# mmSir/SpatioTemporalEntropyModel

Measured on AMD Instinct MI355X. Metric: frames/s, higher is better.
Workload: dtype f32; 1 GPU; configs[1]: SpatioTemporalPriorModel_Res(256,192) training step on mbt2018(192,192) latents, 16 septuplets x 7 frames x 256x256 per GPU, EMLoss, clip 1.0 + Adam 1e-4 / aux Adam 1e-3; per_gpu_batch=16, global_batch=16, parallelism=dp1, stream_priorities=latents=0,side=-1,compute=-1, stream_cu_masks=latents=block:160, plan_selectors=library defaults

## Files before the change

### spatiotemporalentropymodel_amd/csrc/conv_f16x3.hip

```cpp
#include <math.h>
#include <stdlib.h>

#include <type_traits>

#include "f16x3_tail.h"

namespace {

constexpr int XP = BN + 4;
constexpr int imax(int a, int b) { return a > b ? a : b; }
constexpr int lds_stages(int depth) { return depth == 3 ? 3 : 2; }
constexpr int lds_taps(int bm, int depth) { return imax(imax(lds_stages(depth) * NPL * (bm + BN) * 64, 6 * NPL * bm * 64 + NPL * BN * 64), bm * XP * 4); }
constexpr int lds_total(int bm, int depth) { return lds_taps(bm, depth) + 32 * 4; }

struct Fx3Phase {
    int ntaps, S;
    int dy0, dx0;
    int wofs;
    int cps, nsplit;
    int wsofs;
    int ooy, oox;
};

struct Fx3Args {
// ... 17 lines not shown
    float *ws;
    int *cnt;
    int nsplit, cps;
    int xpix;
    signed char dy[MAXTAP], dx[MAXTAP];
    int ptiles, btaps, OHf, OWf;
    Fx3Phase ph[4];
};

#define TAP_OFFSET(t) (tw_first + ((t) / tw_S) * tw_line + ((t) % tw_S) * tw_col)
#define TAP_WALK_NEXT()                                                                         \
    do {                                                                                        \
        const bool wrap_ = pf_t + 1 == tw_T, rowend_ = pf_ts + 1 == tw_S;                       \
        ++pf_q;                                                                                 \
        pf_to = wrap_ ? tw_first : pf_to + (rowend_ ? tw_line - (tw_S - 1) * tw_col : tw_col);  \
        pf_ts = (wrap_ || rowend_) ? 0 : pf_ts + 1;                                             \
        pf_t = wrap_ ? 0 : pf_t + 1;                                                            \
        pf_kc += wrap_ ? 1 : 0;                                                                 \
    } while (0)


__device__ inline int pi4(int x) { return (0x78 >> (2 * x)) & 3; }

template <int BM, int DEPTH, int MS>
__global__ __launch_bounds__(BM * 4) void conv_f16x3_kernel(const Fx3Args a)
{
    static_assert(DEPTH == 2 || DEPTH == 3, "two or three LDS stages");
    static_assert(MS == 32 || (MS == 16 && DEPTH == 3), "the 16-row MFMA shape exists for the three-stage loop");
    constexpr int NSET = 2;
    constexpr int NT = BM * 4;
    constexpr int A_PLANE = BM * 64, A_BUF = NPL * A_PLANE;
    constexpr int PL = NPL;
    constexpr int WPIECES = PL * BN * 4;
    constexpr int BP = (WPIECES + NT - 1) / NT;
    extern __shared__ __attribute__((aligned(16))) unsigned char smem[];
    constexpr int NST = lds_stages(DEPTH);
    unsigned char *As = smem;
    unsigned char *Bs = smem + NST * A_BUF;

    const int tid = threadIdx.x, lane = tid & 63, wave = tid >> 6;
    const int Mtot = a.B * a.OH * a.OW;
    int tile_m = blockIdx.x;
    {
        const int nb = gridDim.x, qq = nb >> 3, rr = nb & 7, xcd = tile_m & 7, idx = tile_m >> 3;
        if (nb >= 16) tile_m = (xcd < rr ? xcd * (qq + 1) : rr * (qq + 1) + (xcd - rr) * qq) + idx;
    }
    const int bm0 = tile_m * BM;
    const int nslab = a.C / KC, pixbytes = nslab * SLAB;

    const int srow = tid >> 2, scol = tid & 3;
    int pb;
    unsigned pmask = 0;
    {
        const int m = bm0 + srow;
        const bool ok = m < Mtot;
        const int mm = ok ? m : 0;
        const int ohw = a.OH * a.OW, b = mm / ohw, rem = mm - b * ohw, qy = rem / a.OW, qx = rem - qy * a.OW;
        const int by = qy * a.stride, bx = qx * a.stride;
        pb = ((b * a.H + by) * a.W + bx) * pixbytes + scol * 16;
        for (int t = 0; t < a.ntaps; ++t) {
            const int iy = by + a.dy[t], ix = bx + a.dx[t];
            if (ok && iy >= 0 && iy < a.H && ix >= 0 && ix < a.W) pmask |= 1u << t;
        }
    }
    const int a_st = srow * 64 + ((scol ^ ((srow >> 2) & 3)) << 4);
    constexpr int WFULL = WPIECES / NT;
    const int wv0 = tid * 16, wvl = WFULL * NT + tid < WPIECES ? (WFULL * NT + tid) * 16 : OOR;
    const int nchunks = a.ntaps * nslab;
    const int q_last = nchunks - 1;
    __syncthreads();

    const __amdgpu_buffer_rsrc_t rx = __builtin_amdgcn_make_buffer_rsrc(const_cast<void *>(a.xp), 0, a.xbytes, 0x00020000);
    const __amdgpu_buffer_rsrc_t rw = __builtin_amdgcn_make_buffer_rsrc(const_cast<void *>(a.wp), 0, a.wbytes, 0x00020000);

    f32x4 rsa[NSET][PL], rsb[NSET][BP];
    auto gload = [&](int t, int tA, int kc, int q, f32x4 (&ra)[PL], f32x4 (&rb)[BP]) {
        const int sA = kc * SLAB, sB = q * B_BUF;
        const int mk = __builtin_amdgcn_sbfe((int)pmask, (unsigned)t, 1u);
        const int off = ((pb + tA) & mk) | (OOR & ~mk);
#pragma unroll
        for (int pl = 0; pl < PL; ++pl) ra[pl] = __builtin_bit_cast(f32x4, __builtin_amdgcn_raw_buffer_load_b128(rx, off + pl * 64, sA, 0));
#pragma unroll
        for (int j = 0; j < WFULL; ++j)
            rb[j] = __builtin_bit_cast(f32x4, __builtin_amdgcn_raw_buffer_load_b128(rw, wv0 + j * (NT * 16), sB, 0));
        if (BP > WFULL) rb[BP - 1] = __builtin_bit_cast(f32x4, __builtin_amdgcn_raw_buffer_load_b128(rw, wvl, sB, 0));
    };
    auto sstore = [&](int buf, f32x4 (&ra)[PL], f32x4 (&rb)[BP]) {
#pragma unroll
        for (int pl = 0; pl < PL; ++pl) *reinterpret_cast<f32x4 *>(As + buf * A_BUF + pl * A_PLANE + a_st) = ra[pl];
#pragma unroll
        for (int j = 0; j < WFULL; ++j) *reinterpret_cast<f32x4 *>(Bs + buf * B_BUF + j * (NT * 16) + tid * 16) = rb[j];
        if (BP > WFULL && WFULL * NT + tid < WPIECES) *reinterpret_cast<f32x4 *>(Bs + buf * B_BUF + (WFULL * NT + tid) * 16) = rb[BP - 1];
    };

    const int wm0 = (wave >> 1) * 32, wn0 = (wave & 1) * 96;
    const int lr = lane & 31, lh = lane >> 5;
    const int sw = (lr >> 2) & 3;
    const int rdA = (wm0 + lr) * 64, rdB = (wn0 + lr) * 64;
    const int pk0 = ((0 + lh) ^ sw) << 4, pk1 = ((2 + lh) ^ sw) << 4;
    const int l16 = lane & 15, lq = lane >> 4;
    const int cm = 4 * pi4(l16 >> 2) + (l16 & 3), rq = 4 * pi4(lq);
    const int rdA16 = (wm0 + cm) * 64 + ((lq ^ pi4(l16 >> 2)) << 4), rdB16 = (wn0 + cm) * 64 + ((lq ^ pi4(l16 >> 2)) << 4);
    auto ROWL = [&](int r) { return MS == 32 ? wm0 + (r & 3) + 8 * (r >> 2) + 4 * lh : wm0 + ((r >> 2) & 1) * 16 + rq + (r & 3); };
    auto COLL = [&](int j, int r) { return MS == 32 ? wn0 + j * 32 + lr : wn0 + j * 32 + (r >> 3) * 16 + cm; };
    f32x16 acc[3];
#pragma unroll
    for (int j = 0; j < 3; ++j)
#pragma unroll
        for (int r = 0; r < 16; ++r) acc[j][r] = 0.f;

    int pf_q = 0, pf_t = 0, pf_kc = 0, pf_ts = 0, pf_to = 0;
    const int tw_T = a.ntaps, tw_S = a.S, tw_col = pixbytes, tw_line = a.W * pixbytes, tw_first = (a.dy[0] * a.W + a.dx[0]) * pixbytes;
    auto step = [&](int cur, f32x4 (&ra)[PL], f32x4 (&rb)[BP]) {
        const unsigned char *Ab = As + cur * A_BUF + rdA, *Bb = Bs + cur * B_BUF + rdB;
        const int t = __builtin_amdgcn_readfirstlane(pf_t), kc = __builtin_amdgcn_readfirstlane(pf_kc), q = __builtin_amdgcn_readfirstlane(pf_q);
        const int to = __builtin_amdgcn_readfirstlane(pf_to);
#pragma unroll
        for (int ks = 0; ks < 2; ++ks) {
            const int pk = ks ? pk1 : pk0;
            h16x8 af[PL], bf[PL][3];
#pragma unroll
            for (int pl = 0; pl < PL; ++pl) af[pl] = *reinterpret_cast<const h16x8 *>(Ab + pl * A_PLANE + pk);
#pragma unroll
            for (int pl = 0; pl < PL; ++pl)
#pragma unroll
                for (int j = 0; j < 3; ++j) bf[pl][j] = *reinterpret_cast<const h16x8 *>(Bb + pl * B_PLANE + j * 32 * 64 + pk);
#pragma unroll
            for (int j = 0; j < 3; ++j) {
                acc[j] = STEM_MFMA16(af[1], bf[0][j], acc[j]);
                acc[j] = STEM_MFMA16(af[0], bf[1][j], acc[j]);
                acc[j] = STEM_MFMA16(af[0], bf[0][j], acc[j]);
            }
            if (ks == 0)
                sstore(cur ^ 1, ra, rb);
            else
                gload(t, to, kc, q, ra, rb);
        }
        if (pf_q < q_last) TAP_WALK_NEXT();
    };
    h16x8 f0a[PL], f0b[PL][3], f1a[PL], f1b[PL][3];
    auto lfrag = [&](int stage, int pk, h16x8 (&af)[PL], h16x8 (&bf)[PL][3]) {
        const unsigned char *Ab = As + stage * A_BUF + rdA + pk, *Bb = Bs + stage * B_BUF + rdB + pk;
        af[1] = *reinterpret_cast<const h16x8 *>(Ab + A_PLANE);
        bf[0][0] = *reinterpret_cast<const h16x8 *>(Bb);
        af[0] = *reinterpret_cast<const h16x8 *>(Ab);
        bf[1][0] = *reinterpret_cast<const h16x8 *>(Bb + B_PLANE);
#pragma unroll
        for (int j = 1; j < 3; ++j) {
            bf[0][j] = *reinterpret_cast<const h16x8 *>(Bb + j * 32 * 64);
            bf[1][j] = *reinterpret_cast<const h16x8 *>(Bb + B_PLANE + j * 32 * 64);
        }
    };
    auto mfma9 = [&](h16x8 (&af)[PL], h16x8 (&bf)[PL][3]) {
#pragma unroll
        for (int j = 0; j < 3; ++j) {
            acc[j] = STEM_MFMA16(af[1], bf[0][j], acc[j]);
            acc[j] = STEM_MFMA16(af[0], bf[1][j], acc[j]);
            acc[j] = STEM_MFMA16(af[0], bf[0][j], acc[j]);
        }
    };
    auto step3 = [&](int rd, int nx, int wr, f32x4 (&ra)[PL], f32x4 (&rb)[BP]) {
        const int t = __builtin_amdgcn_readfirstlane(pf_t), kc = __builtin_amdgcn_readfirstlane(pf_kc), q = __builtin_amdgcn_readfirstlane(pf_q);
        const int to = __builtin_amdgcn_readfirstlane(pf_to);
        lfrag(rd, pk1, f1a, f1b);
        mfma9(f0a, f0b);
        sstore(wr, ra, rb);
        lfrag(nx, pk0, f0a, f0b);
        mfma9(f1a, f1b);
        gload(t, to, kc, q, ra, rb);
#pragma unroll
        for (int i = 0; i < 8; ++i) {
            __builtin_amdgcn_sched_group_barrier(0x008, 1, 0);
            __builtin_amdgcn_sched_group_barrier(0x100, 1, 0);
        }
        __builtin_amdgcn_sched_group_barrier(0x008, 1, 0);
        constexpr int NW = PL + BP;
        __builtin_amdgcn_sched_group_barrier(0x008, 1, 0);
        __builtin_amdgcn_sched_group_barrier(0x200, (NW + 3) / 4, 0);
        __builtin_amdgcn_sched_group_barrier(0x008, 1, 0);
        __builtin_amdgcn_sched_group_barrier(0x200, (NW + 2) / 4, 0);
        __builtin_amdgcn_sched_group_barrier(0x008, 1, 0);
        __builtin_amdgcn_sched_group_barrier(0x200, (NW + 1) / 4, 0);
        __builtin_amdgcn_sched_group_barrier(0x008, 1, 0);
        __builtin_amdgcn_sched_group_barrier(0x200, NW / 4, 0);
#pragma unroll
        for (int i = 0; i < 4; ++i) {
            __builtin_amdgcn_sched_group_barrier(0x008, 1, 0);
            __builtin_amdgcn_sched_group_barrier(0x100, 2, 0);
        }
        __builtin_amdgcn_sched_group_barrier(0x008, 1, 0);
        __builtin_amdgcn_sched_group_barrier(0x020, PL + BP, 0);
        if (pf_q < q_last) TAP_WALK_NEXT();
    };

    h16x8 ga[2][2][PL], gb0[3][PL], gb1[3][PL];
    f32x4 a16[2][6];
    if constexpr (MS == 16) {
#pragma unroll
        for (int mi = 0; mi < 2; ++mi)
#pragma unroll
            for (int nj = 0; nj < 6; ++nj) a16[mi][nj] = f32x4{0.f, 0.f, 0.f, 0.f};
    }
    auto lfragA16 = [&](const unsigned char *base, h16x8 (&A)[2][PL]) {
#pragma unroll
        for (int mi = 0; mi < 2; ++mi)
#pragma unroll
            for (int pl = 0; pl < PL; ++pl) A[mi][pl] = *reinterpret_cast<const h16x8 *>(base + rdA16 + mi * 16 * 64 + pl * A_PLANE);
    };
    auto lfragB16 = [&](const unsigned char *base, int half, h16x8 (&B)[3][PL]) {
#pragma unroll
        for (int n3 = 0; n3 < 3; ++n3)
#pragma unroll
            for (int pl = 0; pl < PL; ++pl) B[n3][pl] = *reinterpret_cast<const h16x8 *>(base + rdB16 + (half * 3 + n3) * 16 * 64 + pl * B_PLANE);
    };
    auto mma18 = [&](h16x8 (&A)[2][PL], h16x8 (&B)[3][PL], int half, f32x4 (&d)[2][6]) {
#pragma unroll
        for (int prod = 0; prod < 3; ++prod)
#pragma unroll
            for (int n3 = 0; n3 < 3; ++n3)
#pragma unroll
                for (int mi = 0; mi < 2; ++mi)
                    d[mi][half * 3 + n3] = __builtin_amdgcn_mfma_f32_16x16x32_f16(A[mi][prod == 0 ? 1 : 0], B[n3][prod == 1 ? 1 : 0],
                                                                                   d[mi][half * 3 + n3], 0, 0, 0);
    };
    auto step3_16 = [&](int rd, int nx, int wr, f32x4 (&ra)[PL], f32x4 (&rb)[BP], h16x8 (&Acur)[2][PL], h16x8 (&Anext)[2][PL]) {
        const int t = __builtin_amdgcn_readfirstlane(pf_t), kc = __builtin_amdgcn_readfirstlane(pf_kc), q = __builtin_amdgcn_readfirstlane(pf_q);
        const int to = __builtin_amdgcn_readfirstlane(pf_to);
        lfragB16(Bs + rd * B_BUF, 1, gb1);
        mma18(Acur, gb0, 0, a16);
        sstore(wr, ra, rb);
        lfragA16(As + nx * A_BUF, Anext);
        lfragB16(Bs + nx * B_BUF, 0, gb0);
        mma18(Acur, gb1, 1, a16);
        gload(t, to, kc, q, ra, rb);
#pragma unroll
        for (int i = 0; i < 6; ++i) {
            __builtin_amdgcn_sched_group_barrier(0x008, 3, 0);
            __builtin_amdgcn_sched_group_barrier(0x100, 1, 0);
        }
        constexpr int NW = PL + BP;
        __builtin_amdgcn_sched_group_barrier(0x008, 2, 0);
        __builtin_amdgcn_sched_group_barrier(0x200, (NW + 3) / 4, 0);
        __builtin_amdgcn_sched_group_barrier(0x008, 2, 0);
        __builtin_amdgcn_sched_group_barrier(0x200, (NW + 2) / 4, 0);
        __builtin_amdgcn_sched_group_barrier(0x008, 2, 0);
        __builtin_amdgcn_sched_group_barrier(0x200, (NW + 1) / 4, 0);
        __builtin_amdgcn_sched_group_barrier(0x008, 2, 0);
        __builtin_amdgcn_sched_group_barrier(0x200, NW / 4, 0);
#pragma unroll
        for (int i = 0; i < 5; ++i) {
            __builtin_amdgcn_sched_group_barrier(0x008, 2, 0);
            __builtin_amdgcn_sched_group_barrier(0x100, 2, 0);
        }
        __builtin_amdgcn_sched_group_barrier(0x020, PL + BP, 0);
        if (pf_q < q_last) TAP_WALK_NEXT();
    };

    auto chunk_of = [&](int q, int &t, int &kc) {
        q = q < q_last ? q : q_last;
        kc = q / a.ntaps;
        t = q - kc * a.ntaps;
        return q;
    };
    {
        int t, kc, q;
        constexpr int PRE = NST - 1;
#pragma unroll
        for (int c = 0; c < PRE; ++c) {
            q = chunk_of(c, t, kc);
            gload(t, TAP_OFFSET(t), kc, q, rsa[0], rsb[0]);
            sstore(c, rsa[0], rsb[0]);
        }
#pragma unroll
        for (int s = 0; s < NSET; ++s) {
            q = chunk_of(PRE + s, t, kc);
            gload(t, TAP_OFFSET(t), kc, q, rsa[s], rsb[s]);
        }
        pf_q = chunk_of(PRE + NSET, pf_t, pf_kc);
        pf_ts = pf_t % tw_S;
        pf_to = TAP_OFFSET(pf_t);
    }
    __shared__ float qred[16];
    const float fac = q_inv(a.xq) * q_inv(a.wq);
    float oscale = 1.f;
    if (a.yp) {
        const float xmax = q_amax(a.xq, qred), wmax = q_amax(a.wq, qred);
        float bm = 0.f, btm = 3.0e38f;
        for (int n = tid; n < a.N; n += NT) {
            if (a.bias) bm = fmaxf(bm, fabsf(a.bias[n]));
            if (a.fuse) {
                const float bb = fmaxf(a.beta[n], a.beta_bound);
                btm = fminf(btm, bb * bb - 1.4551915228366852e-11f);
            }
        }
        bm = block_max(bm, qred);
        float ob = (float)(a.C * a.ntaps) * xmax * wmax + bm;
        if (a.fuse) ob *= __builtin_amdgcn_rsqf(fmaxf(-block_max(-btm, qred), 1e-30f));
        const int oe = q_exp(ob);
        oscale = q_pow2(oe);
        if (blockIdx.x == 0 && tid == 0) a.yq[1] = q_pow2(-oe);
    }
    __syncthreads();
    if constexpr (MS == 16) {
        int rd = 0, nx = 1, wr = 2;
        lfragA16(As, ga[0]);
        lfragB16(Bs, 0, gb0);
        int q = 0;
        for (; q + 1 < nchunks; q += 2) {
            step3_16(rd, nx, wr, rsa[0], rsb[0], ga[0], ga[1]);
            __syncthreads();
            step3_16(nx, wr, rd, rsa[1], rsb[1], ga[1], ga[0]);
            __syncthreads();
            const int o = rd;
            rd = wr; wr = nx; nx = o;
        }
        if (q < nchunks) {
            step3_16(rd, nx, wr, rsa[0], rsb[0], ga[0], ga[1]);
            __syncthreads();
        }
#pragma unroll
        for (int j = 0; j < 3; ++j)
#pragma unroll
            for (int r = 0; r < 16; ++r) acc[j][r] = a16[(r >> 2) & 1][2 * j + (r >> 3)][r & 3];
    } else if constexpr (DEPTH == 3) {
        int rd = 0, nx = 1, wr = 2;
        lfrag(0, pk0, f0a, f0b);
        int q = 0;
        for (; q + 1 < nchunks; q += 2) {
#pragma unroll
            for (int s = 0; s < 2; ++s) {
                step3(rd, nx, wr, rsa[s], rsb[s]);
                __syncthreads();
                const int o = rd;
                rd = nx; nx = wr; wr = o;
            }
        }
        if (q < nchunks) {
            step3(rd, nx, wr, rsa[0], rsb[0]);
            __syncthreads();
        }
    } else {
        int q = 0;
        for (; q + 1 < nchunks; q += 2) {
#pragma unroll
            for (int s = 0; s < 2; ++s) {
                step(s, rsa[s], rsb[s]);
                __syncthreads();
            }
        }
        if (q < nchunks) {
            step(0, rsa[0], rsb[0]);
            __syncthreads();
        }
    }

    float *X2 = reinterpret_cast<float *>(smem);
    float omax = 0.f;
#pragma unroll
    for (int j = 0; j < 3; ++j) {
        float bias2[2];
#pragma unroll
        for (int h = 0; h < 2; ++h) {
            const int n = COLL(j, h * 8);
            bias2[h] = (a.bias && n < a.N) ? a.bias[n] : 0.f;
        }
#pragma unroll
        for (int r = 0; r < 16; ++r) acc[j][r] = acc[j][r] * fac + bias2[r >> 3];
        if (a.epi == 1) {
#pragma unroll
            for (int r = 0; r < 16; ++r) acc[j][r] = acc[j][r] > 0.f ? acc[j][r] : acc[j][r] * a.slope;
        }
    }
    if (a.fuse) {
        float vm = 0.f;
#pragma unroll
        for (int j = 0; j < 3; ++j)
#pragma unroll
// ... 13 lines not shown
                const int m = ROWL(r), c = COLL(j, r) & 31;
                const float t = acc[j][r] * vs;
                hp_t h0, h1;
                q_split(t * t, 1.f, h0, h1);
                unsigned char *d = Sq + slab * (NPL * A_PLANE) + m * 64 + ((((c >> 3) ^ ((m >> 2) & 3)) << 4) | ((c & 7) << 1));
                *reinterpret_cast<hp_t *>(d) = h0;
                *reinterpret_cast<hp_t *>(d + A_PLANE) = h1;
            }
        }
        f32x16 nrm[3];
#pragma unroll
        for (int j = 0; j < 3; ++j)
#pragma unroll
            for (int r = 0; r < 16; ++r) nrm[j][r] = 0.f;
        f32x4 n16[2][6];
#pragma unroll
        for (int mi = 0; mi < 2; ++mi)
#pragma unroll
            for (int nj = 0; nj < 6; ++nj) n16[mi][nj] = f32x4{0.f, 0.f, 0.f, 0.f};
        const __amdgpu_buffer_rsrc_t rg = __builtin_amdgcn_make_buffer_rsrc(const_cast<void *>(a.gp), 0, a.gbytes, 0x00020000);
        f32x4 gb[BP];
        auto gload_g = [&](int kc) {
#pragma unroll
            for (int u = 0; u < WFULL; ++u) gb[u] = __builtin_bit_cast(f32x4, __builtin_amdgcn_raw_buffer_load_b128(rg, wv0 + u * (NT * 16), kc * B_BUF, 0));
            if (BP > WFULL) gb[BP - 1] = __builtin_bit_cast(f32x4, __builtin_amdgcn_raw_buffer_load_b128(rg, wvl, kc * B_BUF, 0));
        };
        gload_g(0);
        for (int kc = 0; kc < nkg; ++kc) {
            __syncthreads();
#pragma unroll
            for (int u = 0; u < WFULL; ++u) *reinterpret_cast<f32x4 *>(Bg + u * (NT * 16) + tid * 16) = gb[u];
            if (BP > WFULL && WFULL * NT + tid < WPIECES) *reinterpret_cast<f32x4 *>(Bg + (WFULL * NT + tid) * 16) = gb[BP - 1];
            __syncthreads();
            if (kc + 1 < nkg) gload_g(kc + 1);
            if constexpr (MS == 16) {
                h16x8 A[2][PL], B0[3][PL], B1[3][PL];
                lfragA16(Sq + kc * (NPL * A_PLANE), A);
                lfragB16(Bg, 0, B0);
                lfragB16(Bg, 1, B1);
                mma18(A, B0, 0, n16);
                mma18(A, B1, 1, n16);
                continue;
            }
            const unsigned char *Ab = Sq + kc * (NPL * A_PLANE) + rdA, *Bb = Bg + rdB;
#pragma unroll
            for (int ks = 0; ks < 2; ++ks) {
                const int pk = ks ? pk1 : pk0;
                h16x8 af[NPL], bf[NPL][3];
#pragma unroll
                for (int pl = 0; pl < NPL; ++pl) af[pl] = *reinterpret_cast<const h16x8 *>(Ab + pl * A_PLANE + pk);
#pragma unroll
                for (int pl = 0; pl < NPL; ++pl)
#pragma unroll
                    for (int j = 0; j < 3; ++j) bf[pl][j] = *reinterpret_cast<const h16x8 *>(Bb + pl * B_PLANE + j * 32 * 64 + pk);
#pragma unroll
// ... 84 lines not shown
        phase = blockIdx.x / a.ptiles;
        bxt = blockIdx.x - phase * a.ptiles;
    }
    const int ntaps = PH ? a.ph[phase].ntaps : a.ntaps, tapS = PH ? a.ph[phase].S : a.S;
    const int cps = PH ? a.ph[phase].cps : a.cps, nsplit = PH ? a.ph[phase].nsplit : a.nsplit;
    const int pdy0 = PH ? a.ph[phase].dy0 : (int)a.dy[0], pdx0 = PH ? a.ph[phase].dx0 : (int)a.dx[0];
    const int wofs = PH ? a.ph[phase].wofs : 0;
    if constexpr (PH) {
        if ((int)blockIdx.z >= nsplit) return;
    }
    float *const wsb = PH ? a.ws + a.ph[phase].wsofs : a.ws;
    constexpr int GNT = GBM * 4, GA_PLANE = GBM * 64, GA_BUF = NPL * GA_PLANE;
    constexpr int PL = NPL, BPC = NPL * GBN * 4 / GNT;
    extern __shared__ __attribute__((aligned(16))) unsigned char smem[];
    unsigned char *As = smem;
    unsigned char *Bs = smem + 2 * GA_BUF;
    int *tapi = reinterpret_cast<int *>(smem + glds_main(GBM));

    const int tid = threadIdx.x, lane = tid & 63, wave = tid >> 6;
    const int Mtot = a.B * a.OH * a.OW;
    const int bm0 = bxt * GBM, bn0 = blockIdx.y * GBN, zsplit = blockIdx.z;
    const int nslab = a.C / KC, pixbytes = a.xpix;

    const int srow = tid >> 2, scol = tid & 3;
    int pb;
    unsigned pmask = 0;
    {
        const int m = bm0 + srow;
        const bool ok = m < Mtot;
        const int mm = ok ? m : 0;
        const int ohw = a.OH * a.OW, b = mm / ohw, rem = mm - b * ohw, qy = rem / a.OW, qx = rem - qy * a.OW;
        const int by = qy * a.stride, bx = qx * a.stride;
        pb = ((b * a.H + by) * a.W + bx) * pixbytes + scol * 16;
        for (int t = 0; t < ntaps; ++t) {
            const int iy = by + (PH ? pdy0 + t / tapS : (int)a.dy[t]), ix = bx + (PH ? pdx0 + t % tapS : (int)a.dx[t]);
            if (ok && iy >= 0 && iy < a.H && ix >= 0 && ix < a.W) pmask |= 1u << t;
        }
    }
    const int a_st = srow * 64 + ((scol ^ ((srow >> 2) & 3)) << 4);
    const int nchunks = ntaps * nslab;
    const int q_begin = zsplit * cps;
    const int q_end = q_begin + cps < nchunks ? q_begin + cps : nchunks;
    const int q_last = q_end - 1;
    const int wbase = blockIdx.y * nchunks;
    __syncthreads();

    const __amdgpu_buffer_rsrc_t rx = __builtin_amdgcn_make_buffer_rsrc(const_cast<void *>(a.xp), 0, a.xbytes, 0x00020000);
    const __amdgpu_buffer_rsrc_t rw = __builtin_amdgcn_make_buffer_rsrc(const_cast<void *>(a.wp), 0, a.wbytes, 0x00020000);

    f32x4 raA[PL], rbA[BPC], raB[PL], rbB[BPC];
    auto gload = [&](int t, int tA, int kc, int q, f32x4 (&ra)[PL], f32x4 (&rb)[BPC]) {
        const int sA = kc * SLAB, sB = wofs + (wbase + q) * GB_BUF;
        const int mk = __builtin_amdgcn_sbfe((int)pmask, (unsigned)t, 1u);
        const int off = ((pb + tA) & mk) | (OOR & ~mk);
#pragma unroll
        for (int pl = 0; pl < PL; ++pl) ra[pl] = __builtin_bit_cast(f32x4, __builtin_amdgcn_raw_buffer_load_b128(rx, off + pl * 64, sA, 0));
#pragma unroll
        for (int j = 0; j < BPC; ++j) rb[j] = __builtin_bit_cast(f32x4, __builtin_amdgcn_raw_buffer_load_b128(rw, tid * 16 + j * (GNT * 16), sB, 0));
    };
    auto sstore = [&](int buf, f32x4 (&ra)[PL], f32x4 (&rb)[BPC]) {
#pragma unroll
        for (int pl = 0; pl < PL; ++pl) *reinterpret_cast<f32x4 *>(As + buf * GA_BUF + pl * GA_PLANE + a_st) = ra[pl];
#pragma unroll
        for (int j = 0; j < BPC; ++j) *reinterpret_cast<f32x4 *>(Bs + buf * GB_BUF + j * (GNT * 16) + tid * 16) = rb[j];
    };

    const int wm0 = (wave >> 1) * 32, wn0 = (wave & 1) * 64;
    const int lr = lane & 31, lh = lane >> 5;
    const int sw = (lr >> 2) & 3;
    const int rdA = (wm0 + lr) * 64, rdB = (wn0 + lr) * 64;
    const int pk0 = ((0 + lh) ^ sw) << 4, pk1 = ((2 + lh) ^ sw) << 4;
    const int l16 = lane & 15, lq = lane >> 4;
    const int cm = 4 * pi4(l16 >> 2) + (l16 & 3), rq = 4 * pi4(lq);
    const int rdA16 = (wm0 + cm) * 64 + ((lq ^ pi4(l16 >> 2)) << 4), rdB16 = (wn0 + cm) * 64 + ((lq ^ pi4(l16 >> 2)) << 4);
    auto ROWL = [&](int r) { return MS == 32 ? wm0 + (r & 3) + 8 * (r >> 2) + 4 * lh : wm0 + ((r >> 2) & 1) * 16 + rq + (r & 3); };
    auto COLL = [&](int j, int r) { return MS == 32 ? wn0 + j * 32 + lr : wn0 + j * 32 + (r >> 3) * 16 + cm; };
    f32x16 acc[2];
#pragma unroll
    for (int j = 0; j < 2; ++j)
#pragma unroll
        for (int r = 0; r < 16; ++r) acc[j][r] = 0.f;

    int pf_q = 0, pf_t = 0, pf_kc = 0, pf_ts = 0, pf_to = 0;
    const int tw_T = ntaps, tw_S = tapS, tw_col = pixbytes, tw_line = a.W * pixbytes, tw_first = (pdy0 * a.W + pdx0) * pixbytes;
    auto step = [&](int cur, f32x4 (&ra)[PL], f32x4 (&rb)[BPC]) {
        const unsigned char *Ab = As + cur * GA_BUF + rdA, *Bb = Bs + cur * GB_BUF + rdB;
        const int t = __builtin_amdgcn_readfirstlane(pf_t), kc = __builtin_amdgcn_readfirstlane(pf_kc), q = __builtin_amdgcn_readfirstlane(pf_q);
        const int to = __builtin_amdgcn_readfirstlane(pf_to);
#pragma unroll
        for (int ks = 0; ks < 2; ++ks) {
            const int pk = ks ? pk1 : pk0;
            h16x8 af[PL], bf[PL][2];
#pragma unroll
            for (int pl = 0; pl < PL; ++pl) af[pl] = *reinterpret_cast<const h16x8 *>(Ab + pl * GA_PLANE + pk);
#pragma unroll
            for (int pl = 0; pl < PL; ++pl)
#pragma unroll
                for (int j = 0; j < 2; ++j) bf[pl][j] = *reinterpret_cast<const h16x8 *>(Bb + pl * GB_PLANE + j * 32 * 64 + pk);
#pragma unroll
            for (int j = 0; j < 2; ++j) {
                acc[j] = STEM_MFMA16(af[1], bf[0][j], acc[j]);
                acc[j] = STEM_MFMA16(af[0], bf[1][j], acc[j]);
                acc[j] = STEM_MFMA16(af[0], bf[0][j], acc[j]);
            }
            if (ks == 0)
                sstore(cur ^ 1, ra, rb);
            else
                gload(t, to, kc, q, ra, rb);
        }
        if (pf_q < q_last) TAP_WALK_NEXT();
    };
    f32x4 a16[2][4];
    if constexpr (MS == 16) {
#pragma unroll
        for (int mi = 0; mi < 2; ++mi)
#pragma unroll
            for (int nj = 0; nj < 4; ++nj) a16[mi][nj] = f32x4{0.f, 0.f, 0.f, 0.f};
    }
    auto step16 = [&](int cur, f32x4 (&ra)[PL], f32x4 (&rb)[BPC]) {
        const unsigned char *Ab = As + cur * GA_BUF + rdA16, *Bb = Bs + cur * GB_BUF + rdB16;
        const int t = __builtin_amdgcn_readfirstlane(pf_t), kc = __builtin_amdgcn_readfirstlane(pf_kc), q = __builtin_amdgcn_readfirstlane(pf_q);
        const int to = __builtin_amdgcn_readfirstlane(pf_to);
        h16x8 A[2][PL], B[4][PL];
#pragma unroll
        for (int mi = 0; mi < 2; ++mi)
#pragma unroll
            for (int pl = 0; pl < PL; ++pl) A[mi][pl] = *reinterpret_cast<const h16x8 *>(Ab + mi * 16 * 64 + pl * GA_PLANE);
#pragma unroll
        for (int nj = 0; nj < 4; ++nj)
#pragma unroll
            for (int pl = 0; pl < PL; ++pl) B[nj][pl] = *reinterpret_cast<const h16x8 *>(Bb + nj * 16 * 64 + pl * GB_PLANE);
#pragma unroll
        for (int prod = 0; prod < 3; ++prod) {
#pragma unroll
            for (int nj = 0; nj < 4; ++nj)
#pragma unroll
                for (int mi = 0; mi < 2; ++mi)
                    a16[mi][nj] = __builtin_amdgcn_mfma_f32_16x16x32_f16(A[mi][prod == 0 ? 1 : 0], B[nj][prod == 1 ? 1 : 0], a16[mi][nj], 0, 0, 0);
            if (prod == 0) sstore(cur ^ 1, ra, rb);
        }
        gload(t, to, kc, q, ra, rb);
        if (pf_q < q_last) TAP_WALK_NEXT();
    };
    const bool dead = bn0 + wn0 >= a.N;
    auto step_dead = [&](int cur, f32x4 (&ra)[PL], f32x4 (&rb)[BPC]) {
        const int t = __builtin_amdgcn_readfirstlane(pf_t), kc = __builtin_amdgcn_readfirstlane(pf_kc), q = __builtin_amdgcn_readfirstlane(pf_q);
        const int to = __builtin_amdgcn_readfirstlane(pf_to);
        sstore(cur ^ 1, ra, rb);
        gload(t, to, kc, q, ra, rb);
        if (pf_q < q_last) TAP_WALK_NEXT();
    };
    auto chunk_of = [&](int q, int &t, int &kc) {
        q = q < q_last ? q : q_last;
        kc = q / ntaps;
        t = q - kc * ntaps;
        return q;
    };
    if (q_begin < q_end) {
        int t, kc, q;
        q = chunk_of(q_begin, t, kc);
        gload(t, TAP_OFFSET(t), kc, q, raA, rbA);
        sstore(0, raA, rbA);
        q = chunk_of(q_begin + 1, t, kc);
        gload(t, TAP_OFFSET(t), kc, q, raA, rbA);
        q = chunk_of(q_begin + 2, t, kc);
        gload(t, TAP_OFFSET(t), kc, q, raB, rbB);
        pf_q = chunk_of(q_begin + 3, pf_t, pf_kc);
        pf_ts = pf_t % tw_S;
        pf_to = TAP_OFFSET(pf_t);
    }
    __shared__ float qred[16];
    const float fac = q_inv(a.xq) * q_inv(a.wq);
    const float oscale = tail_oscale<GNT>(a.yp != nullptr, a.xq, a.wq, a.bias, a.N, a.C * (PH ? a.btaps : ntaps), a.yq, blockIdx.x == 0 && blockIdx.y == 0, qred);
    __syncthreads();
    if (!dead && MS == 16) {
        int q = q_begin;
        for (; q + 1 < q_end; q += 2) {
            step16(0, raA, rbA);
            __syncthreads();
            step16(1, raB, rbB);
            __syncthreads();
        }
        if (q < q_end) {
            step16(0, raA, rbA);
            __syncthreads();
        }
#pragma unroll
        for (int j = 0; j < 2; ++j)
#pragma unroll
            for (int r = 0; r < 16; ++r) acc[j][r] = a16[(r >> 2) & 1][2 * j + (r >> 3)][r & 3];
    } else if (!dead) {
        int q = q_begin;
        for (; q + 1 < q_end; q += 2) {
            step(0, raA, rbA);
            __syncthreads();
            step(1, raB, rbB);
            __syncthreads();
        }
        if (q < q_end) {
            step(0, raA, rbA);
            __syncthreads();
        }
    } else {
        int q = q_begin;
        for (; q + 1 < q_end; q += 2) {
            step_dead(0, raA, rbA);
            __syncthreads();
            step_dead(1, raB, rbB);
            __syncthreads();
        }
        if (q < q_end) {
            step_dead(0, raA, rbA);
            __syncthreads();
        }
    }

    float *T = reinterpret_cast<float *>(smem);
    const int Npad = gridDim.y * GBN;
    constexpr int ERS = GNT / 32, ER = GBM / ERS;
    const int ec4 = tid & 31, er0 = tid >> 5;
    f32x4 ev[ER];
    auto OROW = [&](int row) -> long {
        const int m = bm0 + row;
        if (m >= Mtot) return -1;
        if constexpr (!PH) return m;
        const int ohw = a.OH * a.OW, b = m / ohw, rem = m - b * ohw, qy = rem / a.OW, qx = rem - qy * a.OW;
        const int oy = 2 * qy + a.ph[phase].ooy, ox = 2 * qx + a.ph[phase].oox;
        return oy < a.OHf && ox < a.OWf ? ((long)b * a.OHf + oy) * a.OWf + ox : -1;
    };
    if (nsplit > 1) {
        float *wsp = wsb + (size_t)zsplit * Mtot * Npad;
#pragma unroll
        for (int j = 0; j < 2; ++j) {
#pragma unroll
            for (int r = 0; r < 16; ++r) {
                const int m = bm0 + ROWL(r), n = bn0 + COLL(j, r);
                if (m < Mtot) __hip_atomic_store(&wsp[(size_t)m * Npad + n], acc[j][r], __ATOMIC_RELAXED, __HIP_MEMORY_SCOPE_AGENT);
// ... 382 lines not shown
```

Before: 10280 frames/s.

## Load conv operand chunks straight into LDS with buffer_load lds DMA

Result: faster. 10430 frames/s (median of 6 runs) (+1.4%).

```diff
diff --git a/spatiotemporalentropymodel_amd/csrc/conv_f16x3.hip b/spatiotemporalentropymodel_amd/csrc/conv_f16x3.hip
--- a/spatiotemporalentropymodel_amd/csrc/conv_f16x3.hip
+++ b/spatiotemporalentropymodel_amd/csrc/conv_f16x3.hip
@@ -63,17 +63,36 @@
 
 __device__ inline int pi4(int x) { return (0x78 >> (2 * x)) & 3; }
 
+typedef int rsrc4 __attribute__((ext_vector_type(4)));
+__device__ inline rsrc4 dma_rsrc(const void *p, int bytes)
+{
+    const unsigned long long v = reinterpret_cast<unsigned long long>(p);
+    return rsrc4{(int)(unsigned)v, (int)(unsigned)(v >> 32), bytes, 0x00020000};
+}
+__device__ inline void dma16(const rsrc4 r, unsigned lds_base, int voff, int soff)
+{
+    asm volatile("s_mov_b32 m0, %0\n\ts_nop 0\n\tbuffer_load_dwordx4 %1, %2, %3 offen lds" ::"s"(lds_base), "v"(voff), "s"(r), "s"(soff) : "memory");
+}
+#define DMA_WAIT_BARRIER(n) asm volatile("s_waitcnt vmcnt(%0)\n\ts_barrier" ::"n"(n) : "memory")
+#define LDS_READS_DONE()                            \
+    do {                                            \
+        __builtin_amdgcn_sched_barrier(0);          \
+        __builtin_amdgcn_s_waitcnt(0xC07F);         \
+        __builtin_amdgcn_sched_barrier(0);          \
+    } while (0)
+
 template <int BM, int DEPTH, int MS>
 __global__ __launch_bounds__(BM * 4) void conv_f16x3_kernel(const Fx3Args a)
 {
     static_assert(DEPTH == 2 || DEPTH == 3, "two or three LDS stages");
     static_assert(MS == 32 || (MS == 16 && DEPTH == 3), "the 16-row MFMA shape exists for the three-stage loop");
-    constexpr int NSET = 2;
     constexpr int NT = BM * 4;
     constexpr int A_PLANE = BM * 64, A_BUF = NPL * A_PLANE;
     constexpr int PL = NPL;
     constexpr int WPIECES = PL * BN * 4;
-    constexpr int BP = (WPIECES + NT - 1) / NT;
+    static_assert(WPIECES % NT == 0, "every wavefront copies whole 1 KiB pieces of the weight chunk");
+    constexpr int BP = WPIECES / NT;
+    constexpr int NI = PL + BP;
     extern __shared__ __attribute__((aligned(16))) unsigned char smem[];
     constexpr int NST = lds_stages(DEPTH);
     unsigned char *As = smem;
@@ -89,7 +108,7 @@
     const int bm0 = tile_m * BM;
     const int nslab = a.C / KC, pixbytes = nslab * SLAB;
 
-    const int srow = tid >> 2, scol = tid & 3;
+    const int srow = tid >> 2, scol = (tid & 3) ^ ((srow >> 2) & 3);
     int pb;
     unsigned pmask = 0;
     {
@@ -104,35 +123,28 @@
             if (ok && iy >= 0 && iy < a.H && ix >= 0 && ix < a.W) pmask |= 1u << t;
         }
     }
-    const int a_st = srow * 64 + ((scol ^ ((srow >> 2) & 3)) << 4);
-    constexpr int WFULL = WPIECES / NT;
-    const int wv0 = tid * 16, wvl = WFULL * NT + tid < WPIECES ? (WFULL * NT + tid) * 16 : OOR;
+    const int wv0 = tid * 16;
     const int nchunks = a.ntaps * nslab;
     const int q_last = nchunks - 1;
     __syncthreads();
 
-    const __amdgpu_buffer_rsrc_t rx = __builtin_amdgcn_make_buffer_rsrc(const_cast<void *>(a.xp), 0, a.xbytes, 0x00020000);
-    const __amdgpu_buffer_rsrc_t rw = __builtin_amdgcn_make_buffer_rsrc(const_cast<void *>(a.wp), 0, a.wbytes, 0x00020000);
-
-    f32x4 rsa[NSET][PL], rsb[NSET][BP];
-    auto gload = [&](int t, int tA, int kc, int q, f32x4 (&ra)[PL], f32x4 (&rb)[BP]) {
+    const rsrc4 rx = dma_rsrc(a.xp, a.xbytes), rw = dma_rsrc(a.wp, a.wbytes);
+    const unsigned lds0 = (unsigned)(unsigned long long)(__attribute__((address_space(3))) unsigned char *)smem;
+    const unsigned ldsw = __builtin_amdgcn_readfirstlane(lds0 + wave * 1024);
+    auto dma_range = [&](int stage, int t, int tA, int kc, int q, int lo, int hi) {
         const int sA = kc * SLAB, sB = q * B_BUF;
         const int mk = __builtin_amdgcn_sbfe((int)pmask, (unsigned)t, 1u);
         const int off = ((pb + tA) & mk) | (OOR & ~mk);
-#pragma unroll
-        for (int pl = 0; pl < PL; ++pl) ra[pl] = __builtin_bit_cast(f32x4, __builtin_amdgcn_raw_buffer_load_b128(rx, off + pl * 64, sA, 0));
-#pragma unroll
-        for (int j = 0; j < WFULL; ++j)
-            rb[j] = __builtin_bit_cast(f32x4, __builtin_amdgcn_raw_buffer_load_b128(rw, wv0 + j * (NT * 16), sB, 0));
-        if (BP > WFULL) rb[BP - 1] = __builtin_bit_cast(f32x4, __builtin_amdgcn_raw_buffer_load_b128(rw, wvl, sB, 0));
-    };
-    auto sstore = [&](int buf, f32x4 (&ra)[PL], f32x4 (&rb)[BP]) {
-#pragma unroll
-        for (int pl = 0; pl < PL; ++pl) *reinterpret_cast<f32x4 *>(As + buf * A_BUF + pl * A_PLANE + a_st) = ra[pl];
-#pragma unroll
-        for (int j = 0; j < WFULL; ++j) *reinterpret_cast<f32x4 *>(Bs + buf * B_BUF + j * (NT * 16) + tid * 16) = rb[j];
-        if (BP > WFULL && WFULL * NT + tid < WPIECES) *reinterpret_cast<f32x4 *>(Bs + buf * B_BUF + (WFULL * NT + tid) * 16) = rb[BP - 1];
-    };
+        const unsigned la = ldsw + stage * A_BUF, lb = ldsw + NST * A_BUF + stage * B_BUF;
+#pragma unroll
+        for (int i = lo; i < hi; ++i) {
+            if (i < PL)
+                dma16(rx, la + i * A_PLANE, off + i * 64, sA);
+            else
+                dma16(rw, lb + (i - PL) * (NT * 16), wv0 + (i - PL) * (NT * 16), sB);
+        }
+    };
+    auto dma = [&](int stage, int t, int tA, int kc, int q) { dma_range(stage, t, tA, kc, q, 0, NI); };
 
     const int wm0 = (wave >> 1) * 32, wn0 = (wave & 1) * 96;
     const int lr = lane & 31, lh = lane >> 5;
@@ -152,10 +164,11 @@
 
     int pf_q = 0, pf_t = 0, pf_kc = 0, pf_ts = 0, pf_to = 0;
     const int tw_T = a.ntaps, tw_S = a.S, tw_col = pixbytes, tw_line = a.W * pixbytes, tw_first = (a.dy[0] * a.W + a.dx[0]) * pixbytes;
-    auto step = [&](int cur, f32x4 (&ra)[PL], f32x4 (&rb)[BP]) {
+    auto step = [&](int cur) {
         const unsigned char *Ab = As + cur * A_BUF + rdA, *Bb = Bs + cur * B_BUF + rdB;
         const int t = __builtin_amdgcn_readfirstlane(pf_t), kc = __builtin_amdgcn_readfirstlane(pf_kc), q = __builtin_amdgcn_readfirstlane(pf_q);
         const int to = __builtin_amdgcn_readfirstlane(pf_to);
+        dma(cur ^ 1, t, to, kc, q);
 #pragma unroll
         for (int ks = 0; ks < 2; ++ks) {
             const int pk = ks ? pk1 : pk0;
@@ -172,12 +185,9 @@
                 acc[j] = STEM_MFMA16(af[0], bf[1][j], acc[j]);
                 acc[j] = STEM_MFMA16(af[0], bf[0][j], acc[j]);
             }
-            if (ks == 0)
-                sstore(cur ^ 1, ra, rb);
-            else
-                gload(t, to, kc, q, ra, rb);
         }
         if (pf_q < q_last) TAP_WALK_NEXT();
+        DMA_WAIT_BARRIER(0);
     };
     h16x8 f0a[PL], f0b[PL][3], f1a[PL], f1b[PL][3];
     auto lfrag = [&](int stage, int pk, h16x8 (&af)[PL], h16x8 (&bf)[PL][3]) {
@@ -200,37 +210,35 @@
             acc[j] = STEM_MFMA16(af[0], bf[0][j], acc[j]);
         }
     };
-    auto step3 = [&](int rd, int nx, int wr, f32x4 (&ra)[PL], f32x4 (&rb)[BP]) {
+    auto step3 = [&](int rd, int nx) {
         const int t = __builtin_amdgcn_readfirstlane(pf_t), kc = __builtin_amdgcn_readfirstlane(pf_kc), q = __builtin_amdgcn_readfirstlane(pf_q);
         const int to = __builtin_amdgcn_readfirstlane(pf_to);
         lfrag(rd, pk1, f1a, f1b);
         mfma9(f0a, f0b);
-        sstore(wr, ra, rb);
-        lfrag(nx, pk0, f0a, f0b);
-        mfma9(f1a, f1b);
-        gload(t, to, kc, q, ra, rb);
 #pragma unroll
         for (int i = 0; i < 8; ++i) {
             __builtin_amdgcn_sched_group_barrier(0x008, 1, 0);
             __builtin_amdgcn_sched_group_barrier(0x100, 1, 0);
         }
         __builtin_amdgcn_sched_group_barrier(0x008, 1, 0);
-        constexpr int NW = PL + BP;
-        __builtin_amdgcn_sched_group_barrier(0x008, 1, 0);
-        __builtin_amdgcn_sched_group_barrier(0x200, (NW + 3) / 4, 0);
-        __builtin_amdgcn_sched_group_barrier(0x008, 1, 0);
-        __builtin_amdgcn_sched_group_barrier(0x200, (NW + 2) / 4, 0);
-        __builtin_amdgcn_sched_group_barrier(0x008, 1, 0);
-        __builtin_amdgcn_sched_group_barrier(0x200, (NW + 1) / 4, 0);
-        __builtin_amdgcn_sched_group_barrier(0x008, 1, 0);
-        __builtin_amdgcn_sched_group_barrier(0x200, NW / 4, 0);
-#pragma unroll
-        for (int i = 0; i < 4; ++i) {
+        LDS_READS_DONE();
+        DMA_WAIT_BARRIER(NI);
+        static_assert(NI <= 8, "one copy instruction per MFMA of the second half");
+        const unsigned char *Ab = As + nx * A_BUF + rdA + pk0, *Bb = Bs + nx * B_BUF + rdB + pk0;
+#pragma unroll
+        for (int i = 0; i < 9; ++i) {
+            const int j = i / 3, k = i % 3;
+            if (i < NI) dma_range(rd, t, to, kc, q, i, i + 1);
+            if (i == 0) f0a[1] = *reinterpret_cast<const h16x8 *>(Ab + A_PLANE);
+            if (i == 1) f0b[0][0] = *reinterpret_cast<const h16x8 *>(Bb);
+            if (i == 2) f0a[0] = *reinterpret_cast<const h16x8 *>(Ab);
+            if (i == 3) f0b[1][0] = *reinterpret_cast<const h16x8 *>(Bb + B_PLANE);
+            if (i >= 4 && i < 8) f0b[i & 1][(i - 2) >> 1] = *reinterpret_cast<const h16x8 *>(Bb + (i & 1) * B_PLANE + ((i - 2) >> 1) * 32 * 64);
+            acc[j] = STEM_MFMA16(k == 0 ? f1a[1] : f1a[0], k == 1 ? f1b[1][j] : f1b[0][j], acc[j]);
+            if (i < 8) __builtin_amdgcn_sched_group_barrier(0x100, 1, 0);
             __builtin_amdgcn_sched_group_barrier(0x008, 1, 0);
-            __builtin_amdgcn_sched_group_barrier(0x100, 2, 0);
-        }
-        __builtin_amdgcn_sched_group_barrier(0x008, 1, 0);
-        __builtin_amdgcn_sched_group_barrier(0x020, PL + BP, 0);
+        }
+        LDS_READS_DONE();
         if (pf_q < q_last) TAP_WALK_NEXT();
     };
 
@@ -264,36 +272,45 @@
                     d[mi][half * 3 + n3] = __builtin_amdgcn_mfma_f32_16x16x32_f16(A[mi][prod == 0 ? 1 : 0], B[n3][prod == 1 ? 1 : 0],
                                                                                    d[mi][half * 3 + n3], 0, 0, 0);
     };
-    auto step3_16 = [&](int rd, int nx, int wr, f32x4 (&ra)[PL], f32x4 (&rb)[BP], h16x8 (&Acur)[2][PL], h16x8 (&Anext)[2][PL]) {
+    auto step3_16 = [&](int rd, int nx, h16x8 (&Acur)[2][PL], h16x8 (&Anext)[2][PL]) {
         const int t = __builtin_amdgcn_readfirstlane(pf_t), kc = __builtin_amdgcn_readfirstlane(pf_kc), q = __builtin_amdgcn_readfirstlane(pf_q);
         const int to = __builtin_amdgcn_readfirstlane(pf_to);
         lfragB16(Bs + rd * B_BUF, 1, gb1);
         mma18(Acur, gb0, 0, a16);
-        sstore(wr, ra, rb);
-        lfragA16(As + nx * A_BUF, Anext);
-        lfragB16(Bs + nx * B_BUF, 0, gb0);
-        mma18(Acur, gb1, 1, a16);
-        gload(t, to, kc, q, ra, rb);
 #pragma unroll
         for (int i = 0; i < 6; ++i) {
-            __builtin_amdgcn_sched_group_barrier(0x008, 3, 0);
+            __builtin_amdgcn_sched_group_barrier(0x008, 2, 0);
             __builtin_amdgcn_sched_group_barrier(0x100, 1, 0);
         }
-        constexpr int NW = PL + BP;
-        __builtin_amdgcn_sched_group_barrier(0x008, 2, 0);
-        __builtin_amdgcn_sched_group_barrier(0x200, (NW + 3) / 4, 0);
-        __builtin_amdgcn_sched_group_barrier(0x008, 2, 0);
-        __builtin_amdgcn_sched_group_barrier(0x200, (NW + 2) / 4, 0);
-        __builtin_amdgcn_sched_group_barrier(0x008, 2, 0);
-        __builtin_amdgcn_sched_group_barrier(0x200, (NW + 1) / 4, 0);
-        __builtin_amdgcn_sched_group_barrier(0x008, 2, 0);
-        __builtin_amdgcn_sched_group_barrier(0x200, NW / 4, 0);
-#pragma unroll
-        for (int i = 0; i < 5; ++i) {
-            __builtin_amdgcn_sched_group_barrier(0x008, 2, 0);
-            __builtin_amdgcn_sched_group_barrier(0x100, 2, 0);
-        }
-        __builtin_amdgcn_sched_group_barrier(0x020, PL + BP, 0);
+        __builtin_amdgcn_sched_group_barrier(0x008, 6, 0);
+        LDS_READS_DONE();
+        DMA_WAIT_BARRIER(NI);
+        auto ygroup = [&](auto group_tag) {
+            constexpr int g = decltype(group_tag)::value;
+            constexpr int r0 = g < 2 ? 3 * g : g < 4 ? 2 * g + 2 : 10, r1 = g < 1 ? 3 : g < 3 ? 2 * g + 4 : 10;
+            constexpr int m0 = (g * 18 + 4) / 5, m1 = ((g + 1) * 18 + 4) / 5;
+            dma_range(rd, t, to, kc, q, (g * NI + 4) / 5, ((g + 1) * NI + 4) / 5);
+#pragma unroll
+            for (int r = r0; r < r1; ++r) {
+                if (r < 4)
+                    Anext[r >> 1][r & 1] = *reinterpret_cast<const h16x8 *>(As + nx * A_BUF + rdA16 + (r >> 1) * 16 * 64 + (r & 1) * A_PLANE);
+                else
+                    gb0[(r - 4) >> 1][r & 1] = *reinterpret_cast<const h16x8 *>(Bs + nx * B_BUF + rdB16 + ((r - 4) >> 1) * 16 * 64 + (r & 1) * B_PLANE);
+            }
+#pragma unroll
+            for (int m = m0; m < m1; ++m) {
+                const int prod = m / 6, n3 = (m % 6) >> 1, mi = m & 1;
+                a16[mi][3 + n3] = __builtin_amdgcn_mfma_f32_16x16x32_f16(Acur[mi][prod == 0 ? 1 : 0], gb1[n3][prod == 1 ? 1 : 0], a16[mi][3 + n3], 0, 0, 0);
+            }
+            if constexpr (r1 > r0) __builtin_amdgcn_sched_group_barrier(0x100, r1 - r0, 0);
+            __builtin_amdgcn_sched_group_barrier(0x008, m1 - m0, 0);
+        };
+        ygroup(std::integral_constant<int, 0>{});
+        ygroup(std::integral_constant<int, 1>{});
+        ygroup(std::integral_constant<int, 2>{});
+        ygroup(std::integral_constant<int, 3>{});
+        ygroup(std::integral_constant<int, 4>{});
+        LDS_READS_DONE();
         if (pf_q < q_last) TAP_WALK_NEXT();
     };
 
@@ -305,19 +322,13 @@
     };
     {
         int t, kc, q;
-        constexpr int PRE = NST - 1;
+        constexpr int PRE = DEPTH == 3 ? 3 : 1;
 #pragma unroll
         for (int c = 0; c < PRE; ++c) {
             q = chunk_of(c, t, kc);
-            gload(t, TAP_OFFSET(t), kc, q, rsa[0], rsb[0]);
-            sstore(c, rsa[0], rsb[0]);
-        }
-#pragma unroll
-        for (int s = 0; s < NSET; ++s) {
-            q = chunk_of(PRE + s, t, kc);
-            gload(t, TAP_OFFSET(t), kc, q, rsa[s], rsb[s]);
-        }
-        pf_q = chunk_of(PRE + NSET, pf_t, pf_kc);
+            dma(c, t, TAP_OFFSET(t), kc, q);
+        }
+        pf_q = chunk_of(PRE, pf_t, pf_kc);
         pf_ts = pf_t % tw_S;
         pf_to = TAP_OFFSET(pf_t);
     }
@@ -342,23 +353,20 @@
         if (blockIdx.x == 0 && tid == 0) a.yq[1] = q_pow2(-oe);
     }
     __syncthreads();
+    DMA_WAIT_BARRIER(DEPTH == 3 ? 2 * NI : 0);
     if constexpr (MS == 16) {
         int rd = 0, nx = 1, wr = 2;
         lfragA16(As, ga[0]);
         lfragB16(Bs, 0, gb0);
+        LDS_READS_DONE();
         int q = 0;
         for (; q + 1 < nchunks; q += 2) {
-            step3_16(rd, nx, wr, rsa[0], rsb[0], ga[0], ga[1]);
-            __syncthreads();
-            step3_16(nx, wr, rd, rsa[1], rsb[1], ga[1], ga[0]);
-            __syncthreads();
+            step3_16(rd, nx, ga[0], ga[1]);
+            step3_16(nx, wr, ga[1], ga[0]);
             const int o = rd;
             rd = wr; wr = nx; nx = o;
         }
-        if (q < nchunks) {
-            step3_16(rd, nx, wr, rsa[0], rsb[0], ga[0], ga[1]);
-            __syncthreads();
-        }
+        if (q < nchunks) step3_16(rd, nx, ga[0], ga[1]);
 #pragma unroll
         for (int j = 0; j < 3; ++j)
 #pragma unroll
@@ -366,34 +374,27 @@
     } else if constexpr (DEPTH == 3) {
         int rd = 0, nx = 1, wr = 2;
         lfrag(0, pk0, f0a, f0b);
+        LDS_READS_DONE();
         int q = 0;
         for (; q + 1 < nchunks; q += 2) {
 #pragma unroll
             for (int s = 0; s < 2; ++s) {
-                step3(rd, nx, wr, rsa[s], rsb[s]);
-                __syncthreads();
+                step3(rd, nx);
                 const int o = rd;
                 rd = nx; nx = wr; wr = o;
             }
         }
-        if (q < nchunks) {
-            step3(rd, nx, wr, rsa[0], rsb[0]);
-            __syncthreads();
-        }
+        if (q < nchunks) step3(rd, nx);
     } else {
         int q = 0;
         for (; q + 1 < nchunks; q += 2) {
 #pragma unroll
-            for (int s = 0; s < 2; ++s) {
-                step(s, rsa[s], rsb[s]);
-                __syncthreads();
-            }
-        }
-        if (q < nchunks) {
-            step(0, rsa[0], rsb[0]);
-            __syncthreads();
-        }
-    }
+            for (int s = 0; s < 2; ++s) step(s);
+        }
+        if (q < nchunks) step(0);
+    }
+    asm volatile("s_waitcnt vmcnt(0)" ::: "memory");
+    __syncthreads();
 
     float *X2 = reinterpret_cast<float *>(smem);
     float omax = 0.f;
@@ -453,15 +454,13 @@
         f32x4 gb[BP];
         auto gload_g = [&](int kc) {
 #pragma unroll
-            for (int u = 0; u < WFULL; ++u) gb[u] = __builtin_bit_cast(f32x4, __builtin_amdgcn_raw_buffer_load_b128(rg, wv0 + u * (NT * 16), kc * B_BUF, 0));
-            if (BP > WFULL) gb[BP - 1] = __builtin_bit_cast(f32x4, __builtin_amdgcn_raw_buffer_load_b128(rg, wvl, kc * B_BUF, 0));
+            for (int u = 0; u < BP; ++u) gb[u] = __builtin_bit_cast(f32x4, __builtin_amdgcn_raw_buffer_load_b128(rg, wv0 + u * (NT * 16), kc * B_BUF, 0));
         };
         gload_g(0);
         for (int kc = 0; kc < nkg; ++kc) {
             __syncthreads();
 #pragma unroll
-            for (int u = 0; u < WFULL; ++u) *reinterpret_cast<f32x4 *>(Bg + u * (NT * 16) + tid * 16) = gb[u];
-            if (BP > WFULL && WFULL * NT + tid < WPIECES) *reinterpret_cast<f32x4 *>(Bg + (WFULL * NT + tid) * 16) = gb[BP - 1];
+            for (int u = 0; u < BP; ++u) *reinterpret_cast<f32x4 *>(Bg + u * (NT * 16) + tid * 16) = gb[u];
             __syncthreads();
             if (kc + 1 < nkg) gload_g(kc + 1);
             if constexpr (MS == 16) {
@@ -592,7 +591,7 @@
     const int bm0 = bxt * GBM, bn0 = blockIdx.y * GBN, zsplit = blockIdx.z;
     const int nslab = a.C / KC, pixbytes = a.xpix;
 
-    const int srow = tid >> 2, scol = tid & 3;
+    const int srow = tid >> 2, scol = (tid & 3) ^ ((srow >> 2) & 3);
     int pb;
     unsigned pmask = 0;
     {
@@ -607,7 +606,6 @@
             if (ok && iy >= 0 && iy < a.H && ix >= 0 && ix < a.W) pmask |= 1u << t;
         }
     }
-    const int a_st = srow * 64 + ((scol ^ ((srow >> 2) & 3)) << 4);
     const int nchunks = ntaps * nslab;
     const int q_begin = zsplit * cps;
     const int q_end = q_begin + cps < nchunks ? q_begin + cps : nchunks;
@@ -615,24 +613,18 @@
     const int wbase = blockIdx.y * nchunks;
     __syncthreads();
 
-    const __amdgpu_buffer_rsrc_t rx = __builtin_amdgcn_make_buffer_rsrc(const_cast<void *>(a.xp), 0, a.xbytes, 0x00020000);
-    const __amdgpu_buffer_rsrc_t rw = __builtin_amdgcn_make_buffer_rsrc(const_cast<void *>(a.wp), 0, a.wbytes, 0x00020000);
-
-    f32x4 raA[PL], rbA[BPC], raB[PL], rbB[BPC];
-    auto gload = [&](int t, int tA, int kc, int q, f32x4 (&ra)[PL], f32x4 (&rb)[BPC]) {
+    const rsrc4 rx = dma_rsrc(a.xp, a.xbytes), rw = dma_rsrc(a.wp, a.wbytes);
+    const unsigned lds0 = (unsigned)(unsigned long long)(__attribute__((address_space(3))) unsigned char *)smem;
+    const unsigned ldsw = __builtin_amdgcn_readfirstlane(lds0 + wave * 1024);
+    auto dma = [&](int stage, int t, int tA, int kc, int q) {
         const int sA = kc * SLAB, sB = wofs + (wbase + q) * GB_BUF;
         const int mk = __builtin_amdgcn_sbfe((int)pmask, (unsigned)t, 1u);
         const int off = ((pb + tA) & mk) | (OOR & ~mk);
-#pragma unroll
-        for (int pl = 0; pl < PL; ++pl) ra[pl] = __builtin_bit_cast(f32x4, __builtin_amdgcn_raw_buffer_load_b128(rx, off + pl * 64, sA, 0));
-#pragma unroll
-        for (int j = 0; j < BPC; ++j) rb[j] = __builtin_bit_cast(f32x4, __builtin_amdgcn_raw_buffer_load_b128(rw, tid * 16 + j * (GNT * 16), sB, 0));
-    };
-    auto sstore = [&](int buf, f32x4 (&ra)[PL], f32x4 (&rb)[BPC]) {
-#pragma unroll
-        for (int pl = 0; pl < PL; ++pl) *reinterpret_cast<f32x4 *>(As + buf * GA_BUF + pl * GA_PLANE + a_st) = ra[pl];
-#pragma unroll
-        for (int j = 0; j < BPC; ++j) *reinterpret_cast<f32x4 *>(Bs + buf * GB_BUF + j * (GNT * 16) + tid * 16) = rb[j];
+        const unsigned la = ldsw + stage * GA_BUF, lb = ldsw + 2 * GA_BUF + stage * GB_BUF;
+#pragma unroll
+        for (int pl = 0; pl < PL; ++pl) dma16(rx, la + pl * GA_PLANE, off + pl * 64, sA);
+#pragma unroll
+        for (int j = 0; j < BPC; ++j) dma16(rw, lb + j * (GNT * 16), tid * 16 + j * (GNT * 16), sB);
     };
 
     const int wm0 = (wave >> 1) * 32, wn0 = (wave & 1) * 64;
@@ -653,10 +645,11 @@
 
     int pf_q = 0, pf_t = 0, pf_kc = 0, pf_ts = 0, pf_to = 0;
     const int tw_T = ntaps, tw_S = tapS, tw_col = pixbytes, tw_line = a.W * pixbytes, tw_first = (pdy0 * a.W + pdx0) * pixbytes;
-    auto step = [&](int cur, f32x4 (&ra)[PL], f32x4 (&rb)[BPC]) {
+    auto step = [&](int cur) {
         const unsigned char *Ab = As + cur * GA_BUF + rdA, *Bb = Bs + cur * GB_BUF + rdB;
         const int t = __builtin_amdgcn_readfirstlane(pf_t), kc = __builtin_amdgcn_readfirstlane(pf_kc), q = __builtin_amdgcn_readfirstlane(pf_q);
         const int to = __builtin_amdgcn_readfirstlane(pf_to);
+        dma(cur ^ 1, t, to, kc, q);
 #pragma unroll
         for (int ks = 0; ks < 2; ++ks) {
             const int pk = ks ? pk1 : pk0;
@@ -673,12 +666,9 @@
                 acc[j] = STEM_MFMA16(af[0], bf[1][j], acc[j]);
                 acc[j] = STEM_MFMA16(af[0], bf[0][j], acc[j]);
             }
-            if (ks == 0)
-                sstore(cur ^ 1, ra, rb);
-            else
-                gload(t, to, kc, q, ra, rb);
         }
         if (pf_q < q_last) TAP_WALK_NEXT();
+        DMA_WAIT_BARRIER(0);
     };
     f32x4 a16[2][4];
     if constexpr (MS == 16) {
@@ -687,10 +677,11 @@
 #pragma unroll
             for (int nj = 0; nj < 4; ++nj) a16[mi][nj] = f32x4{0.f, 0.f, 0.f, 0.f};
     }
-    auto step16 = [&](int cur, f32x4 (&ra)[PL], f32x4 (&rb)[BPC]) {
+    auto step16 = [&](int cur) {
         const unsigned char *Ab = As + cur * GA_BUF + rdA16, *Bb = Bs + cur * GB_BUF + rdB16;
         const int t = __builtin_amdgcn_readfirstlane(pf_t), kc = __builtin_amdgcn_readfirstlane(pf_kc), q = __builtin_amdgcn_readfirstlane(pf_q);
         const int to = __builtin_amdgcn_readfirstlane(pf_to);
+        dma(cur ^ 1, t, to, kc, q);
         h16x8 A[2][PL], B[4][PL];
 #pragma unroll
         for (int mi = 0; mi < 2; ++mi)
@@ -701,24 +692,22 @@
 #pragma unroll
             for (int pl = 0; pl < PL; ++pl) B[nj][pl] = *reinterpret_cast<const h16x8 *>(Bb + nj * 16 * 64 + pl * GB_PLANE);
 #pragma unroll
-        for (int prod = 0; prod < 3; ++prod) {
+        for (int prod = 0; prod < 3; ++prod)
 #pragma unroll
             for (int nj = 0; nj < 4; ++nj)
 #pragma unroll
                 for (int mi = 0; mi < 2; ++mi)
                     a16[mi][nj] = __builtin_amdgcn_mfma_f32_16x16x32_f16(A[mi][prod == 0 ? 1 : 0], B[nj][prod == 1 ? 1 : 0], a16[mi][nj], 0, 0, 0);
-            if (prod == 0) sstore(cur ^ 1, ra, rb);
-        }
-        gload(t, to, kc, q, ra, rb);
         if (pf_q < q_last) TAP_WALK_NEXT();
+        DMA_WAIT_BARRIER(0);
     };
     const bool dead = bn0 + wn0 >= a.N;
-    auto step_dead = [&](int cur, f32x4 (&ra)[PL], f32x4 (&rb)[BPC]) {
+    auto step_dead = [&](int cur) {
         const int t = __builtin_amdgcn_readfirstlane(pf_t), kc = __builtin_amdgcn_readfirstlane(pf_kc), q = __builtin_amdgcn_readfirstlane(pf_q);
         const int to = __builtin_amdgcn_readfirstlane(pf_to);
-        sstore(cur ^ 1, ra, rb);
-        gload(t, to, kc, q, ra, rb);
+        dma(cur ^ 1, t, to, kc, q);
         if (pf_q < q_last) TAP_WALK_NEXT();
+        DMA_WAIT_BARRIER(0);
     };
     auto chunk_of = [&](int q, int &t, int &kc) {
         q = q < q_last ? q : q_last;
@@ -729,13 +718,8 @@
     if (q_begin < q_end) {
         int t, kc, q;
         q = chunk_of(q_begin, t, kc);
-        gload(t, TAP_OFFSET(t), kc, q, raA, rbA);
-        sstore(0, raA, rbA);
-        q = chunk_of(q_begin + 1, t, kc);
-        gload(t, TAP_OFFSET(t), kc, q, raA, rbA);
-        q = chunk_of(q_begin + 2, t, kc);
-        gload(t, TAP_OFFSET(t), kc, q, raB, rbB);
-        pf_q = chunk_of(q_begin + 3, pf_t, pf_kc);
+        dma(0, t, TAP_OFFSET(t), kc, q);
+        pf_q = chunk_of(q_begin + 1, pf_t, pf_kc);
         pf_ts = pf_t % tw_S;
         pf_to = TAP_OFFSET(pf_t);
     }
@@ -743,18 +727,14 @@
     const float fac = q_inv(a.xq) * q_inv(a.wq);
     const float oscale = tail_oscale<GNT>(a.yp != nullptr, a.xq, a.wq, a.bias, a.N, a.C * (PH ? a.btaps : ntaps), a.yq, blockIdx.x == 0 && blockIdx.y == 0, qred);
     __syncthreads();
+    DMA_WAIT_BARRIER(0);
     if (!dead && MS == 16) {
         int q = q_begin;
         for (; q + 1 < q_end; q += 2) {
-            step16(0, raA, rbA);
-            __syncthreads();
-            step16(1, raB, rbB);
-            __syncthreads();
-        }
-        if (q < q_end) {
-            step16(0, raA, rbA);
-            __syncthreads();
-        }
+            step16(0);
+            step16(1);
+        }
+        if (q < q_end) step16(0);
 #pragma unroll
         for (int j = 0; j < 2; ++j)
 #pragma unroll
@@ -762,27 +742,17 @@
     } else if (!dead) {
         int q = q_begin;
         for (; q + 1 < q_end; q += 2) {
-            step(0, raA, rbA);
-            __syncthreads();
-            step(1, raB, rbB);
-            __syncthreads();
-        }
-        if (q < q_end) {
-            step(0, raA, rbA);
-            __syncthreads();
-        }
+            step(0);
+            step(1);
+        }
+        if (q < q_end) step(0);
     } else {
         int q = q_begin;
         for (; q + 1 < q_end; q += 2) {
-            step_dead(0, raA, rbA);
-            __syncthreads();
-            step_dead(1, raB, rbB);
-            __syncthreads();
-        }
-        if (q < q_end) {
-            step_dead(0, raA, rbA);
-            __syncthreads();
-        }
+            step_dead(0);
+            step_dead(1);
+        }
+        if (q < q_end) step_dead(0);
     }
 
     float *T = reinterpret_cast<float *>(smem);
```
